# xiezhy6/PASTA-GAN-plusplus

Hardware: AMD Instinct MI355X
Metric: 512-res try-on images/sec (SynthesisNetwork fwd) (higher is better)
Workload: dtype f32

## Files before the change

### include/pasta_gan_ops.h

```cpp
#ifndef PASTA_GAN_OPS_H
#define PASTA_GAN_OPS_H

#include <stdint.h>

#ifdef __cplusplus
extern "C" {
#endif

#define PG_ABI_VERSION 19

enum pg_dtype { PG_F32 = 0, PG_F16 = 1, PG_BF16 = 2, PG_F64 = 3 };

enum pg_error {
    PG_OK = 0,
    PG_ERR_INVALID_ARG = -1,
    PG_ERR_UNSUPPORTED = -2,
    PG_ERR_TOO_LARGE = -3
};

enum pg_act {
    PG_ACT_LINEAR = 1, PG_ACT_RELU = 2, PG_ACT_LRELU = 3, PG_ACT_TANH = 4, PG_ACT_SIGMOID = 5,
    PG_ACT_ELU = 6, PG_ACT_SELU = 7, PG_ACT_SOFTPLUS = 8, PG_ACT_SWISH = 9
};

int pg_bias_act(const void* x, const void* b, const void* xref, const void* yref, const void* dy, void* y,
                int dtype, int64_t sizeX, int sizeB, int64_t stepB,
                int grad, int act, float alpha, float gain, float clamp, void* stream);
int pg_bias_act_abi_version(void);

int64_t pg_bias_act_grad_bias_workspace(int dtype, int64_t sizeX, int sizeB, int64_t stepB);
int pg_bias_act_grad_bias(const void* dy, const void* yref, void* dx, void* db, void* workspace, int64_t workspace_bytes,
                          int dtype, int64_t sizeX, int sizeB, int64_t stepB,
                          int act, float alpha, float gain, float clamp, void* stream);

int pg_upfirdn2d(const void* x, const float* f, void* y, int dtype,
                 int N, int C, int inH, int inW, const int64_t xstride[4],
                 int fh, int fw, const int64_t fstride[2],
                 int outH, int outW, const int64_t ystride[4],
                 int upx, int upy, int downx, int downy, int padx0, int pady0,
                 int flip, float gain, void* stream);
int pg_upfirdn2d_with_odd_samples(const void* x, const float* f, void* y, float* y_odd, int dtype,
                                  int N, int C, int inH, int inW, const int64_t xstride[4],
// ... 78 lines not shown
int pg_modconv_prep(const float* w2, const float* styles, float* out, float* s_norm, void* s16, int half_dtype,
                    int N, int Cout, int Cin, int normalize, int demodulate, void* stream);

#define PG_MODCONV_PREP_MAX_JOBS 32
typedef struct {
    const float* w2[PG_MODCONV_PREP_MAX_JOBS];
    const float* styles[PG_MODCONV_PREP_MAX_JOBS];
    float*       out[PG_MODCONV_PREP_MAX_JOBS];
    float*       s_norm[PG_MODCONV_PREP_MAX_JOBS];
    void*        s16[PG_MODCONV_PREP_MAX_JOBS];
    int          cout[PG_MODCONV_PREP_MAX_JOBS];
    int          cin[PG_MODCONV_PREP_MAX_JOBS];
    int          flags[PG_MODCONV_PREP_MAX_JOBS];
    int          njobs;
    int          half_dtype;
} pg_modconv_prep_jobs;
int pg_modconv_prep_batched(const pg_modconv_prep_jobs* jobs, int N, void* stream);

int pg_conv2d_up2_forward(const float* x, const float* packed, float* y, int N, int Cin, int H, int W, int Cout,
                          const int64_t ystride[4], const float* in_scale, const float* out_scale, void* stream);
int pg_conv2d_up2_splitk_plan(int N, int Cin, int H, int W, int Cout);
int pg_conv2d_up2_forward_splitk(const float* x, const float* packed, float* y, int N, int Cin, int H, int W, int Cout,
                                 const int64_t ystride[4], const float* in_scale, const float* out_scale, float* workspace, int ksplit, void* stream);

int64_t pg_conv2d_up2x3_packed_size(int Cout, int Cin);
int pg_conv2d_up2x3_pack_weight(const float* packed, void* packed_x3, int Cout, int Cin, void* stream);
int pg_conv2d_up2x3_forward(const float* x, const float* packed, const void* packed_x3, float* y, int N, int Cin, int H, int W, int Cout,
                            const int64_t ystride[4], const float* in_scale, const float* out_scale, float* edge_column, void* stream);

int64_t pg_conv2d_stem7x3_packed_size(int Cout);
int pg_conv2d_stem7x3_pack_weight(const float* w, void* packed, int Cout, float scale, int flip_hw, void* stream);
int pg_conv2d_stem7x3_forward(const float* x, const void* packed, float* y, int N, int H, int W, int Cout, const int64_t ystride[4],
                              const pg_conv2d_fusion* fusion, void* stream);

int pg_conv1x1_small(const float* x, const float* w, const float* styles, const float* bias, const float* skip, float* y,
                     int N, int Cin, int64_t HW, int Cout, float scale, float clamp, void* stream);

int pg_conv1x1_fold_prep(const float* wm, const float* bm, const float* wh, const float* bh, const float* styles, float* w_out, float* b_out,
                         int N, int Cm, int C, int Cout, void* stream);
int pg_conv1x1_fold_heads(const float* x, const float* x2, const float* w, const float* bias, const float* skip, float* y_a, float* y_b,
                          int N, int C1, int C2, int64_t HW, int Cout, int c_a, int n_skip, float clamp, void* stream);

int pg_conv3x3_fold_head(const float* xa, const float* xb, const float* w, const float* bias, const float* skip, float* y,
                         int N, int C, int H, int W, int Cout, float clamp, void* stream);

int pg_conv3x3_cin1(const float* x, const float* w, float* y, int N, int H, int W, int Cout, float scale, int act, void* stream);

int pg_instance_norm_stats(const float* x, float* mean, float* rstd, int NC, int64_t HW, float eps, void* stream);
int pg_spade_norm(const float* x, const float* mean, const float* rstd, const float* gamma, const float* beta,
                  float* y, int NC, int64_t HW, void* stream);

#define PG_STATS16_MAX_CHUNKS 256
int pg_instance_norm_stats_cl16(const void* x, float* mean, float* rstd, float* workspace, int dtype, int N, int64_t HW, int C, float eps, void* stream);
int pg_spade_combine_cl16(const void* x, const float* mean, const float* rstd, const void* gamma_beta, void* y, int dtype, int N, int64_t HW, int C,
                          int act, float alpha, float gain, float clamp, void* stream);

int pg_spade_train_forward(const float* x, const float* mean, const float* rstd, const float* gamma, const float* beta, float* y,
                           int N, int C, int64_t HW, int64_t gamma_sample_stride, int64_t beta_sample_stride, void* stream);
int pg_spade_train_backward(const float* dy, const float* x, const float* mean, const float* rstd, const float* gamma, float* sums,
                            float* dx, float* dgamma, float* dbeta, int N, int C, int64_t HW,
                            int64_t gamma_sample_stride, int64_t dgamma_sample_stride, int64_t dbeta_sample_stride, void* stream);

int pg_spade_masked_sums(const float* feat, const float* mask, const float* denorm_mask, float* sums, float* counts,
                         int N, int C, int H, int W, void* stream);
int pg_spade_feat_assemble(const float* feat_upper, const float* feat_lower, const float* mask_upper, const float* mask_lower,
                           const float* denorm_mask_upper, const float* denorm_mask_lower,
// ... 251 lines not shown
```

### pasta-gan-plusplus_amd/torch_utils/custom_ops.py

```python

import concurrent.futures
import ctypes
import fcntl
import glob
import hashlib
import os
import re
import shutil
import subprocess
import sys

verbosity = 'brief'

CSRC_DIR = os.path.normpath(os.path.join(os.path.dirname(os.path.abspath(__file__)), '..', 'csrc'))
INCLUDE_DIR = os.path.normpath(os.path.join(CSRC_DIR, '..', '..', 'include'))
DEV_DIR = os.path.join(CSRC_DIR, 'dev')
OFFLOAD_ARCH = 'gfx950'
HIPCC_FLAGS = ['-O3', '-std=c++17', '-fPIC', '-fvisibility=hidden', f'--offload-arch={OFFLOAD_ARCH}']

PLUGIN_SOURCES = {
    'bias_act_plugin': ['bias_act.hip'],
    'upfirdn2d_plugin': ['upfirdn2d.hip'],
    'patch_routing_plugin': ['patch_routing.hip'],
    'augment_plugin': ['augment.hip'],
    'tryon_plugin': ['tryon.hip'],
    'tryon_front_plugin': ['tryon_front.hip'],
    'train_fetch_plugin': ['train_fetch.hip'],
    'snapshot_grid_plugin': ['snapshot_grid.hip'],
    'vgg_loss_plugin': ['vgg_loss.hip'],
    'image_metrics_plugin': ['image_metrics.hip'],
    'conv2d_plugin': ['conv2d.hip', 'conv2d_inst_k3s1.hip', 'conv2d_inst_k1s1.hip', 'conv2d_inst_k2x2.hip', 'conv2d_inst_k2x1.hip',
                      'conv2d_inst_k1x2.hip', 'conv2d_inst_k7s1.hip', 'conv2d_inst_k3s2.hip', 'conv2d_inst_k1s2.hip', 'conv2d_inst_wino.hip', 'conv2d_inst_wino4.hip', 'conv2d_inst_wino4s.hip', 'conv2d_inst_wino4t.hip', 'conv2d_inst_wino4x.hip', 'conv2d_inst_wino4xs.hip', 'conv2d_inst_wino4xt.hip', 'conv2d_inst_wino4b.hip', 'conv2d_inst_wino4bs.hip', 'conv2d_inst_up2.hip', 'conv2d_inst_stem7.hip', 'conv2d_inst_s1x1.hip',
                      'conv2d_wgrad.hip', 'conv2d16.hip', 'conv2d16_inst_k3s1.hip', 'conv2d16_inst_k3s1b.hip', 'conv2d16_inst_k1s1.hip', 'conv2d16_inst_k2x2.hip', 'conv2d16_inst_k2x1.hip',
                      'conv2d16_inst_k1x2.hip', 'conv2d16_inst_k3s2.hip', 'conv2d16_inst_up2f.hip', 'conv1x1_head16.hip', 'spade16.hip', 'conv1x1_fold.hip', 'conv3x3_fold.hip', 'optim.hip'],
}

ABI_VERSION = 19

_cached_plugins = dict()


class NativePlugin:

    def __init__(self, name, path, abi_name=None):
        self.name = name
        self.path = path
        self.lib = ctypes.CDLL(path)
        probe = getattr(self.lib, 'pg_' + (abi_name or name).replace('_plugin', '') + '_abi_version', None)
        if probe is None:
            raise RuntimeError(f'{path} does not export its ABI version; rebuild it from csrc/')
        probe.restype = ctypes.c_int
        if probe() != ABI_VERSION:
            raise RuntimeError(f'{path} implements ABI version {probe()}, the bindings expect {ABI_VERSION}; rebuild it from csrc/')

    def __repr__(self):
        return f'<NativePlugin {self.name} at {self.path}>'


def _find_hipcc():
    for cand in (os.environ.get('HIPCC'), shutil.which('hipcc'), '/opt/rocm/bin/hipcc'):
        if cand and os.path.isfile(cand):
            return cand
    return None


def _digest(sources, extra_flags):
    h = hashlib.md5()
    deps = sorted(set(list(sources) + glob.glob(os.path.join(CSRC_DIR, '*.h')) + glob.glob(os.path.join(INCLUDE_DIR, '*.h'))))
    for path in deps:
        h.update(os.path.basename(path).encode())
# ... 180 lines not shown
```

### pasta-gan-plusplus_amd/torch_utils/ops/conv2d_gradfix.py

```python

import contextlib
import os

import weakref

import torch

from . import _native as nat
from . import bias_act
from . import conv2d_mfma
from . import conv2d_mfma16

native_input_gradients = os.environ.get('PG_NATIVE_DGRAD', '1') == '1'
native_weight_gradients16 = os.environ.get('PG_NATIVE_WGRAD16', '1') == '1'
native_weight_gradients = os.environ.get('PG_NATIVE_WGRAD', '1') == '1'
enabled = True
weight_gradients_disabled = False


@contextlib.contextmanager
def no_weight_gradients():
    global weight_gradients_disabled
    old = weight_gradients_disabled
    weight_gradients_disabled = True
# ... 117 lines not shown
    if hit is None:
        w = weight.detach()
        if not w.is_contiguous():
            w = w.contiguous()
        hit = conv2d_mfma.pack_weight(w, flip=flip, transpose_oi=transpose_oi, winograd=winograd)
        if sum(e[1].numel() * e[1].element_size() for e in _pack_cache.values()) + hit.numel() * hit.element_size() > _PACK_CACHE_MAX_BYTES:
            _pack_cache.clear()

        def _evict(ref, key=key):
            e = _pack_cache.get(key)
            if e is not None and e[0] is ref:
                del _pack_cache[key]
        _pack_cache[key] = (weakref.ref(base, _evict), hit)
    return hit


def _epilogue_backward(ctx, dy, y, ep, want_b):
    act, alpha, gain, clamp = ep
    if want_b:
        return bias_act._BiasActGrad.apply(dy, None, None, y, 1, act, alpha, gain, clamp, True)
    return bias_act._BiasActGrad.apply(dy, None, None, y, 1, act, alpha, gain, clamp), None


class _Conv2dMfma(torch.autograd.Function):
    @staticmethod
    def forward(ctx, x, weight, bias, stride, padding, transposed, output_padding, ep=None):
        x = x.contiguous()
        n, cin, h, w = x.shape
        kh, kw = int(weight.shape[2]), int(weight.shape[3])
        if not transposed:
            cout = int(weight.shape[0])
            fz = dict(act=ep[0], alpha=ep[1], gain=ep[2], clamp=ep[3] if ep[3] >= 0 else None) if ep is not None else {}
            wg = conv2d_mfma.use_winograd(kh, kw, stride, cout, cin, pad=padding, hw=(h, w), ep=fz)
            y = conv2d_mfma.conv2d_forward(x, _packed(weight, wg), cout, kh, kw, stride=stride, pad=padding, bias=bias, winograd=wg, **fz)
        else:
            assert ep is None
            cout = int(weight.shape[1])
            out_hw = ((h - 1) * stride - 2 * padding[0] + kh + output_padding[0], (w - 1) * stride - 2 * padding[1] + kw + output_padding[1])
            if ((kh, kw, stride) == (3, 3, 2) and tuple(padding) == (0, 0) and tuple(output_padding) == (0, 0) and bias is None and UP2_TRANSPOSED
                    and (n * cout * out_hw[0] * ((out_hw[1] + 3) // 4 * 4)) * 4 < 2 ** 31):
                main = _packed(weight, 0, flip=False, transpose_oi=True)
                packs = dict(main=main)
                if UP2_TRANSPOSED_X3 and cin % 16 == 0 and cin >= 32:
                    hit = _x3_of_pack.get(id(main))
                    if hit is None or hit[0]() is not main:
                        x3 = conv2d_mfma.pack_s2x3_planes(main, cout, cin)
                        _x3_of_pack[id(main)] = hit = (weakref.ref(main, lambda r, k=id(main): _x3_of_pack.pop(k, None)), x3)
                    packs['x3'] = hit[1]
                y = conv2d_mfma.conv_up2_forward(x, packs, cout, x3=None if 'x3' in packs else False)
            else:
                phases = conv2d_mfma.pack_transposed(weight, stride, padding, (h, w), out_hw)
                y = conv2d_mfma.conv_transpose2d_forward(x, phases, cout, out_hw, stride=stride, bias=bias)
        ctx.save_for_backward(x, weight, y if ep is not None else None)
        ctx.cfg = (stride, padding, transposed, output_padding, bias is not None, ep)
        return y

    @staticmethod
    def backward(ctx, dy):
        x, weight, y = ctx.saved_tensors
        stride, padding, transposed, output_padding, has_bias, ep = ctx.cfg
        kh, kw = int(weight.shape[2]), int(weight.shape[3])
        dx = dw = db = None
        if ep is not None:
            dy, db = _epilogue_backward(ctx, dy, y, ep, has_bias and ctx.needs_input_grad[2])
        if ctx.needs_input_grad[0] and native_input_gradients:
            dx = _input_gradient(dy, x.shape, weight, stride, padding, transposed, output_padding)
        want_w = ctx.needs_input_grad[1] and not weight_gradients_disabled
# ... 138 lines not shown
```

### pasta-gan-plusplus_amd/torch_utils/ops/conv2d_mfma.py

```python

import contextlib
import ctypes
import os

import torch

from .. import custom_ops
from . import _native as nat

ACT_INDEX = {'linear': 1, 'relu': 2, 'lrelu': 3, 'tanh': 4, 'sigmoid': 5, 'elu': 6, 'selu': 7, 'softplus': 8, 'swish': 9}

FUSED_ACTS = ('linear', 'relu', 'lrelu')

SUPPORTED = {(3, 3, 1), (1, 1, 1), (2, 2, 1), (2, 1, 1), (1, 2, 1), (7, 7, 1), (3, 3, 2), (1, 1, 2)}


class Fusion(ctypes.Structure):
    _fields_ = [
        ('in_scale', ctypes.c_void_p), ('in_bias', ctypes.c_void_p), ('in_act', ctypes.c_int), ('in_alpha', ctypes.c_float),
        ('in_gain', ctypes.c_float), ('in_clamp', ctypes.c_float),
        ('out_scale', ctypes.c_void_p), ('noise', ctypes.c_void_p), ('noise_batch_stride', ctypes.c_int64), ('noise_gain', ctypes.c_float),
        ('bias', ctypes.c_void_p), ('act', ctypes.c_int), ('alpha', ctypes.c_float), ('gain', ctypes.c_float), ('clamp', ctypes.c_float),
        ('residual', ctypes.c_void_p),
        ('spade_x', ctypes.c_void_p), ('spade_mean', ctypes.c_void_p), ('spade_rstd', ctypes.c_void_p),
        ('x2', ctypes.c_void_p), ('cin_split', ctypes.c_int),
        ('stats_partial', ctypes.c_void_p),
    ]


_plugin = None

_timeline = None
_wgrad_timeline = None


def reserve_cus(n):
# ... 71 lines not shown
        lib.pg_spade_norm.argtypes = [vp, vp, vp, vp, vp, vp, i, i64, vp]
        lib.pg_spade_train_forward.restype = i
        lib.pg_spade_train_forward.argtypes = [vp] * 6 + [i, i, i64, i64, i64, vp]
        lib.pg_spade_train_backward.restype = i
        lib.pg_spade_train_backward.argtypes = [vp] * 9 + [i, i, i64, i64, i64, i64, vp]
        lib.pg_conv2d_wgrad_plan.restype = i
        lib.pg_conv2d_wgrad_plan.argtypes = [i] * 8
        lib.pg_conv2d_wgrad.restype = i
        lib.pg_conv2d_wgrad.argtypes = [vp, vp, vp, vp] + [i] * 13 + [vp]
        lib.pg_conv2d_up2_forward.restype = i
        lib.pg_conv2d_up2_forward.argtypes = [vp, vp, vp, i, i, i, i, i, ctypes.POINTER(ctypes.c_int64), vp, vp, vp]
        lib.pg_split3_bf16_cl.restype = i
        lib.pg_split3_bf16_cl.argtypes = [vp, vp, i, i, i64, vp]
        lib.pg_conv2d16_wgrad_x3.restype = i
        lib.pg_conv2d16_wgrad_x3.argtypes = [vp, vp, vp, vp] + [i] * 13 + [vp]
        lib.pg_conv2d16_wgrad_plan.restype = i
        lib.pg_conv2d16_wgrad_plan.argtypes = [i] * 8
        lib.pg_conv2d_up2_splitk_plan.restype = i
        lib.pg_conv2d_up2_splitk_plan.argtypes = [i, i, i, i, i]
        lib.pg_conv2d_up2x3_packed_size.restype = i64
        lib.pg_conv2d_up2x3_packed_size.argtypes = [i, i]
        lib.pg_conv2d_up2x3_pack_weight.restype = i
        lib.pg_conv2d_up2x3_pack_weight.argtypes = [vp, vp, i, i, vp]
        lib.pg_conv2d_up2x3_forward.restype = i
        lib.pg_conv2d_up2x3_forward.argtypes = [vp, vp, vp, vp, i, i, i, i, i, ctypes.POINTER(ctypes.c_int64), vp, vp, vp, vp]
        lib.pg_conv2d_up2_forward_splitk.restype = i
        lib.pg_conv2d_up2_forward_splitk.argtypes = [vp, vp, vp, i, i, i, i, i, ctypes.POINTER(ctypes.c_int64), vp, vp, vp, i, vp]
        lib.pg_conv2d_stem7x3_packed_size.restype = i64
        lib.pg_conv2d_stem7x3_packed_size.argtypes = [i]
        lib.pg_conv2d_stem7x3_pack_weight.restype = i
        lib.pg_conv2d_stem7x3_pack_weight.argtypes = [vp, vp, i, ctypes.c_float, i, vp]
        lib.pg_conv2d_stem7x3_forward.restype = i
        lib.pg_conv2d_stem7x3_forward.argtypes = [vp, vp, vp, i, i, i, i, ctypes.POINTER(ctypes.c_int64), ctypes.POINTER(Fusion), vp]
        lib.pg_conv3x3_cin1.restype = i
        lib.pg_conv3x3_cin1.argtypes = [vp, vp, vp, i, i, i, i, f, i, vp]
        lib.pg_conv1x1_small.restype = i
        lib.pg_conv1x1_small.argtypes = [vp] * 6 + [i, i, i64, i, f, f, vp]
        lib.pg_conv1x1_fold_prep.restype = i
        lib.pg_conv1x1_fold_prep.argtypes = [vp] * 7 + [i, i, i, i, vp]
        lib.pg_conv1x1_fold_heads.restype = i
        lib.pg_conv1x1_fold_heads.argtypes = [vp] * 7 + [i, i, i, i64, i, i, i, f, vp]
        lib.pg_conv3x3_fold_head.restype = i
        lib.pg_conv3x3_fold_head.argtypes = [vp] * 6 + [i, i, i, i, i, f, vp]
        _plugin = plugin
    return _plugin


WINO_F2, WINO_F4, WINO_F4B, WINO_F4X3 = 1, 2, 3, 4
WINO_FORMS = {0: ('direct', False, False), WINO_F2: ('winograd', False, False), WINO_F4: ('winograd4', True, False),
              WINO_F4B: ('winograd4', False, True), WINO_F4X3: ('winograd4x3', True, False)}


def _wino_form(winograd):
    if int(winograd) not in WINO_FORMS:
        raise nat.NativeOpError(f'conv2d_mfma: winograd={winograd!r} is not one of the forms {sorted(WINO_FORMS)}')
    return (int(winograd), *WINO_FORMS[int(winograd)])


_WINO4B = os.environ.get('PG_WINO4B', '1')
F4_FORM = WINO_F4 if _WINO4B == '0' else WINO_F4B
F4_WIDE = WINO_F4 if os.environ.get('PG_WINO4_X3', '1') == '0' else WINO_F4X3


def f4_form(hw):
    if _WINO4B == '2':
        return WINO_F4B
# ... 46 lines not shown


def _f32c(t, name):
    if t is None:
        return None
    if t.dtype != torch.float32 or not t.is_cuda:
        raise nat.NativeOpError(f'conv2d_mfma: {name} must be a float32 GPU tensor')
    return t.contiguous()


def pack_weight(w, scale=1.0, flip=False, transpose_oi=False, winograd=False):
    lib = _init().lib
    w = _f32c(w.detach(), 'weight')
    if transpose_oi:
        cin, cout, kh, kw = w.shape
    else:
        cout, cin, kh, kw = w.shape
    form = _wino_form(winograd)[0]
    if form:
        if (kh, kw) != (3, 3):
            raise nat.NativeOpError('conv2d_mfma: the Winograd layout is for 3x3 weights')
        packed = torch.empty([lib.pg_conv2d_winograd_packed_size(form, cout, cin)], dtype=torch.float32, device=w.device)
        with torch.cuda.device(w.device):
            st = lib.pg_conv2d_winograd_pack_weight(form, nat.ptr(w), nat.ptr(packed), cout, cin, float(scale), int(bool(flip)), int(bool(transpose_oi)), nat.stream_of(w))
        nat.check(st, 'pg_conv2d_winograd_pack_weight')
        return packed
    packed = torch.empty([lib.pg_conv2d_packed_size(cout, cin, kh, kw)], dtype=torch.float32, device=w.device)
    with torch.cuda.device(w.device):
        st = lib.pg_conv2d_pack_weight(nat.ptr(w), nat.ptr(packed), cout, cin, kh, kw, float(scale), int(bool(flip)), int(bool(transpose_oi)), nat.stream_of(w))
    nat.check(st, 'pg_conv2d_pack_weight')
    return packed


def conv2d_forward(x, packed, cout, kh, kw, stride=1, pad=(0, 0), out_hw=None, y=None, out_step=(1, 1), out_off=(0, 0),
                   in_scale=None, in_bias=None, in_act='linear', in_alpha=0.0, in_gain=1.0, in_clamp=None,
                   out_scale=None, noise=None, noise_gain=1.0, bias=None, act='linear', alpha=0.0, gain=1.0, clamp=None,
                   residual=None, spade=None, x2=None, winograd=False, stats_eps=None):
    lib = _init().lib
    form, label, has_stats_tail, _ = _wino_form(winograd)
    x = _f32c(x, 'x')
    n, cin, h, w = x.shape
    cin_split = 0
    if x2 is not None:
        x2 = _f32c(x2, 'x2')
        if x2.shape[0] != n or x2.shape[2:] != x.shape[2:] or cin % 16 != 0:
            raise nat.NativeOpError('conv2d_mfma: x2 must match x in N, H, W and x must have a multiple of 16 channels')
        cin_split, cin = cin, cin + x2.shape[1]
    pad_y, pad_x = pad
    if out_hw is None:
        out_hw = ((h + 2 * pad_y - kh) // stride + 1, (w + 2 * pad_x - kw) // stride + 1)
    oh, ow = out_hw
    ychan = cout // 2 if spade is not None else cout
    if y is None:
        assert tuple(out_step) == (1, 1) and tuple(out_off) == (0, 0)
        y = torch.empty([n, ychan, oh, ow], dtype=torch.float32, device=x.device)
    else:
        assert y.dtype == torch.float32 and y.device == x.device and y.shape[0] == n and y.shape[1] == ychan
    fz = Fusion()
    keep = []

    def dev(t, name, numel=None):
        t = _f32c(t, name)
        if t is None:
            return None
        if numel is not None and t.numel() != numel:
            raise nat.NativeOpError(f'conv2d_mfma: {name} has {t.numel()} elements, expected {numel}')
        keep.append(t)
        return t.data_ptr()

    fz.in_scale = dev(in_scale, 'in_scale', n * cin)
# ... 10 lines not shown
        else:
            raise nat.NativeOpError('conv2d_mfma: noise must have OH*OW or N*OH*OW elements')
        keep.append(noise)
        fz.noise = noise.data_ptr()
    fz.noise_gain = float(noise_gain)
    fz.bias = dev(bias, 'bias', cout)
    fz.act, fz.alpha, fz.gain = ACT_INDEX[act], float(alpha), float(gain)
    fz.clamp = -1.0 if clamp is None else float(clamp)
    if residual is not None:
        if residual.dtype != torch.float32 or residual.shape != y.shape or residual.stride() != y.stride():
            raise nat.NativeOpError('conv2d_mfma: residual must match y in dtype, shape and strides')
        keep.append(residual)
        fz.residual = residual.data_ptr()
    if spade is not None:
        sx, smean, srstd = spade
        if sx.dtype != torch.float32 or sx.shape != y.shape or sx.stride() != y.stride() or smean.numel() != n * ychan or srstd.numel() != n * ychan:
            raise nat.NativeOpError('conv2d_mfma: spade tensors must match the [N, C, OH, OW] output')
        keep += [sx, smean, srstd]
        fz.spade_x, fz.spade_mean, fz.spade_rstd = sx.data_ptr(), smean.data_ptr(), srstd.data_ptr()
    if x2 is not None:
        keep.append(x2)
        fz.x2, fz.cin_split = x2.data_ptr(), cin_split
    stats_part = None
    if stats_eps is not None:
        if not has_stats_tail or spade is not None or in_scale is not None or noise is not None or residual is not None or x2 is not None or in_act != 'linear':
            raise nat.NativeNotCovered('conv2d_mfma: output statistics are gathered by the F(4x4) kernel\'s plain tail only')
        stats_T = lib.pg_conv2d_winograd4_stats_tiles(int(oh), int(ow))
        stats_part = torch.empty([n * cout * stats_T * 2], dtype=torch.float32, device=x.device)
        fz.stats_partial = stats_part.data_ptr()
    with torch.cuda.device(x.device):
        if _timeline is not None:
            ev0, ev1 = torch.cuda.Event(enable_timing=True), torch.cuda.Event(enable_timing=True)
            ev0.record()
        if form:
            if (kh, kw, int(stride)) != (3, 3, 1) or tuple(out_step) != (1, 1) or tuple(out_off) != (0, 0):
                raise nat.NativeOpError('conv2d_mfma: winograd=True needs a 3x3 stride-1 dense-output launch')
            st = lib.pg_conv2d_winograd_forward(form, nat.ptr(x), nat.ptr(packed), nat.ptr(y), n, cin, h, w, cout, int(pad_y), int(pad_x),
                                                int(oh), int(ow), nat.i64arr(y.stride()), ctypes.byref(fz), nat.stream_of(x))
        else:
            ksplit = 1
            if spade is None and x2 is None and os.environ.get('PG_CONV_SPLITK', '1') != '0':
                ksplit = lib.pg_conv2d_splitk_plan(n, cin, int(oh), int(ow), cout, kh, kw, int(stride))
            if ksplit > 1:
                ws = torch.empty([ksplit * n * cout * int(oh) * int(ow)], dtype=torch.float32, device=x.device)
                st = lib.pg_conv2d_forward_splitk(nat.ptr(x), nat.ptr(packed), nat.ptr(y), n, cin, h, w, cout, kh, kw, int(stride), int(pad_y), int(pad_x),
                                                  int(oh), int(ow), nat.i64arr(y.stride()), int(out_step[0]), int(out_step[1]), int(out_off[0]), int(out_off[1]),
                                                  ctypes.byref(fz), nat.ptr(ws), ksplit, nat.stream_of(x))
            else:
                st = lib.pg_conv2d_forward(nat.ptr(x), nat.ptr(packed), nat.ptr(y), n, cin, h, w, cout, kh, kw, int(stride), int(pad_y), int(pad_x),
                                           int(oh), int(ow), nat.i64arr(y.stride()), int(out_step[0]), int(out_step[1]), int(out_off[0]), int(out_off[1]),
                                           ctypes.byref(fz), nat.stream_of(x))
        if _timeline is not None:
            ev1.record()
            _timeline.append(((kh, kw, int(stride), label, f'N{n} {cin}->{cout} {h}x{w}' + (' spade' if spade is not None else '') + (' xf' if in_act != 'linear' else '') + (' mod' if in_scale is not None else '') + (' res' if residual is not None else '')), 2.0 * n * cout * oh * ow * cin * kh * kw, ev0, ev1,
                              4 * (x.numel() + (x2.numel() if x2 is not None else 0) + n * ychan * oh * ow)))
    nat.check(st, 'pg_conv2d_forward')
    if stats_part is not None:
        mean = torch.empty([n * cout], dtype=torch.float32, device=x.device)
        rstd = torch.empty_like(mean)
        with torch.cuda.device(x.device):
            st = lib.pg_instance_norm_finish(nat.ptr(stats_part), nat.ptr(mean), nat.ptr(rstd), n * cout, stats_T, int(oh), int(ow), float(stats_eps), nat.stream_of(x))
        nat.check(st, 'pg_instance_norm_finish')
        return y, (mean, rstd)
    return y


def pack_spade_gamma_beta(w_gamma, w_beta, scale_gamma=1.0, scale_beta=1.0, winograd=False):
    c = int(w_gamma.shape[0])
    grp = 32
    assert w_gamma.shape == w_beta.shape and c % 32 == 0
    if _wino_form(winograd)[3]:
        gw, bw = w_gamma.detach() * scale_gamma, w_beta.detach() * scale_beta
        return pack_weight(torch.stack([gw, bw], dim=1).reshape(2 * c, *w_gamma.shape[1:]).contiguous(), winograd=winograd)
    g = (w_gamma.detach() * scale_gamma).reshape(c // grp, grp, *w_gamma.shape[1:])
    b = (w_beta.detach() * scale_beta).reshape(c // grp, grp, *w_beta.shape[1:])
    return pack_weight(torch.cat([g, b], dim=1).reshape(2 * c, *w_gamma.shape[1:]).contiguous(), winograd=winograd)


def transposed_phases(kh, kw, stride, pad_y, pad_x, in_hw, out_hw):
    s = stride

    def axis(k, pad, n_out):
        res = []
        for a in range(s):
            j = -(-(k - a) // s)
            if j <= 0:
                return None
# ... 521 lines not shown
```

Baseline: 285.0.

## Add warp-specialized bf16x3 MFMA kernel for 3x3 stride-2 unpadded convolutions

Adds a dedicated persistent kernel for 3x3 stride-2 pad-0 convolutions. Producer waves DMA input rows into LDS and split each fp32 value into three bf16 planes, while consumer waves run bf16 32x32x16 MFMAs over six plane products to emulate fp32 precision, with double-buffered planes and prefetched weight slabs. The goal is to move these convs from the generic fp32 path onto the matrix cores. It is used by default only in inference with no grad and simple epilogues, and falls back when unsupported. The bf16x3 split gives slightly different rounding than true fp32.

```diff
diff --git a/include/pasta_gan_ops.h b/include/pasta_gan_ops.h
--- a/include/pasta_gan_ops.h
+++ b/include/pasta_gan_ops.h
@@ -7,7 +7,7 @@
 extern "C" {
 #endif
 
-#define PG_ABI_VERSION 19
+#define PG_ABI_VERSION 20
 
 enum pg_dtype { PG_F32 = 0, PG_F16 = 1, PG_BF16 = 2, PG_F64 = 3 };
 
@@ -152,6 +152,11 @@
 int pg_conv2d_stem7x3_pack_weight(const float* w, void* packed, int Cout, float scale, int flip_hw, void* stream);
 int pg_conv2d_stem7x3_forward(const float* x, const void* packed, float* y, int N, int H, int W, int Cout, const int64_t ystride[4],
                               const pg_conv2d_fusion* fusion, void* stream);
+
+int64_t pg_conv2d_s2x3_packed_size(int Cout, int Cin);
+int pg_conv2d_s2x3_pack_weight(const float* packed, void* packed_x3, int Cout, int Cin, void* stream);
+int pg_conv2d_s2x3_forward(const float* x, const void* packed_x3, float* y, int N, int Cin, int H, int W, int Cout, const int64_t ystride[4],
+                           const pg_conv2d_fusion* fusion, void* stream);
 
 int pg_conv1x1_small(const float* x, const float* w, const float* styles, const float* bias, const float* skip, float* y,
                      int N, int Cin, int64_t HW, int Cout, float scale, float clamp, void* stream);
diff --git a/pasta-gan-plusplus_amd/csrc/conv2d_inst_s2x3.hip b/pasta-gan-plusplus_amd/csrc/conv2d_inst_s2x3.hip
--- /dev/null
+++ b/pasta-gan-plusplus_amd/csrc/conv2d_inst_s2x3.hip
@@ -0,0 +1,38 @@
+#include "conv2d_s2x3.h"
+
+PG_EXPORT int64_t pg_conv2d_s2x3_packed_size(int Cout, int Cin) {
+    if (Cout <= 0 || Cin <= 0 || Cin % 16 != 0) return 0;
+    return pgconv::s2x3_packed_bytes(Cout, Cin);
+}
+
+PG_EXPORT int pg_conv2d_s2x3_pack_weight(const float* packed, void* packed_x3, int Cout, int Cin, void* stream) {
+    if (!packed || !packed_x3 || Cout <= 0 || Cin <= 0 || (((uintptr_t)packed_x3) & 15) != 0) return PG_ERR_INVALID_ARG;
+    if (Cin % 16 != 0) return PG_ERR_UNSUPPORTED;
+    const int CoutP32 = (Cout + 31) / 32 * 32, CoutP128 = (Cout + 127) / 128 * 128;
+    const int64_t total = (int64_t)Cin * 9 * CoutP128;
+    int64_t blocks = (total + 255) / 256;
+    if (blocks > (int64_t)pg::max_stream_blocks()) blocks = pg::max_stream_blocks();
+    hipLaunchKernelGGL(pgconv::s2x3_pack_kernel, dim3((unsigned)blocks), dim3(256), 0, (hipStream_t)stream, packed, (unsigned short*)packed_x3, Cin, CoutP128, CoutP32);
+    return pg::launch_status();
+}
+
+PG_EXPORT int pg_conv2d_s2x3_forward(const float* x, const void* packed_x3, float* y, int N, int Cin, int H, int W, int Cout, const int64_t ystride[4],
+                                     const pg_conv2d_fusion* fusion, void* stream) {
+    if (!x || !packed_x3 || !y || !ystride || N <= 0 || Cin <= 0 || H <= 0 || W <= 0 || Cout <= 0) return PG_ERR_INVALID_ARG;
+    if ((((uintptr_t)x) & 3) != 0 || (((uintptr_t)packed_x3) & 15) != 0) return PG_ERR_INVALID_ARG;
+    pgconv::S2x3Params p;
+    p.x = x; p.y = y; p.wx3 = (const unsigned char*)packed_x3; p.bias = nullptr;
+    p.N = N; p.Cin = Cin; p.H = H; p.W = W; p.Cout = Cout;
+    for (int i = 0; i < 4; i++) p.ys[i] = ystride[i];
+    p.act = PG_ACT_LINEAR; p.alpha = 0.f; p.gain = 1.f; p.clamp = -1.f;
+    if (fusion) {
+        const pg_conv2d_fusion& f = *fusion;
+        if (f.in_scale || f.in_bias || (f.in_act != 0 && f.in_act != PG_ACT_LINEAR) || f.in_clamp >= 0.f || (f.in_gain != 0.f && f.in_gain != 1.f) || f.out_scale || f.noise || f.residual ||
+            f.spade_x || f.spade_mean || f.spade_rstd || f.x2 || f.stats_partial)
+            return PG_ERR_UNSUPPORTED;
+        const int act = f.act == 0 ? PG_ACT_LINEAR : f.act;
+        if (act != PG_ACT_LINEAR && act != PG_ACT_RELU && act != PG_ACT_LRELU) return PG_ERR_UNSUPPORTED;
+        p.bias = f.bias; p.act = act; p.alpha = f.alpha; p.gain = f.gain == 0.f ? 1.f : f.gain; p.clamp = f.clamp;
+    }
+    return pgconv::launch_s2x3(p, (hipStream_t)stream);
+}
diff --git a/pasta-gan-plusplus_amd/csrc/conv2d_s2x3.h b/pasta-gan-plusplus_amd/csrc/conv2d_s2x3.h
--- /dev/null
+++ b/pasta-gan-plusplus_amd/csrc/conv2d_s2x3.h
@@ -0,0 +1,353 @@
+#pragma once
+#include "conv2d_kernel.h"
+
+#ifndef SX_EXP
+#define SX_EXP 0
+#endif
+
+namespace pgconv {
+
+constexpr int SX_KC = 16;
+constexpr int SX_TH = 4, SX_TW = 16;
+constexpr int SX_IH = 9, SX_IW = 33;
+constexpr int SX_RW = 10;
+constexpr int SX_RAW = (512 + 3 * 320) * 4;
+constexpr int SX_PR = 34;
+constexpr int SX_NPIX = SX_IH * SX_PR;
+constexpr int SX_PLB = SX_NPIX * 32;
+constexpr int SX_GROUP = 128;
+constexpr int SX_FRAG = 64 * 16;
+constexpr int SX_WSLAB = 27 * SX_FRAG;
+constexpr size_t SX_LDS = (size_t)SX_RAW * 4 + 2 * 3 * (size_t)SX_PLB + 2 * SX_GROUP * 4;
+
+struct S2x3Params {
+    const float* x; float* y; const unsigned char* wx3; const float* bias;
+    int N, Cin, H, W, Cout, OH, OW;
+    int tilesX, tilesY, groups, total_tiles;
+    int64_t ys[4];
+    int act; float alpha, gain, clamp;
+};
+
+typedef __bf16 sx_bf16x8 __attribute__((ext_vector_type(8)));
+typedef unsigned sx_u32x4 __attribute__((ext_vector_type(4)));
+
+__device__ __forceinline__ void sx_split_pair(float va, float vb, unsigned& p0, unsigned& p1, unsigned& p2) {
+    const unsigned ua = __float_as_uint(va), ub = __float_as_uint(vb);
+    const float ra = va - __uint_as_float(ua & 0xffff0000u), rb = vb - __uint_as_float(ub & 0xffff0000u);
+    const unsigned ura = __float_as_uint(ra), urb = __float_as_uint(rb);
+    const float la = ra - __uint_as_float(ura & 0xffff0000u), lb = rb - __uint_as_float(urb & 0xffff0000u);
+    p0 = __builtin_amdgcn_perm(ub, ua, 0x07060302u);
+    p1 = __builtin_amdgcn_perm(urb, ura, 0x07060302u);
+    p2 = __builtin_amdgcn_perm(__float_as_uint(lb), __float_as_uint(la), 0x07060302u);
+}
+
+__global__ __launch_bounds__(512, 1) void conv2d_s2x3(S2x3Params p) {
+    extern __shared__ __attribute__((aligned(16))) unsigned char sx_smem[];
+    float* raw = (float*)sx_smem;
+    unsigned char* planes = sx_smem + SX_RAW * 4;
+    float* bias_s = (float*)(planes + 2 * 3 * SX_PLB);
+
+    const int wave = __builtin_amdgcn_readfirstlane((int)threadIdx.x >> 6);
+    const int lane = (int)threadIdx.x & 63;
+    const unsigned smem_b = __builtin_amdgcn_readfirstlane(lds_offset((const float*)sx_smem));
+    const int HW = p.H * p.W;
+    const int nchunks = p.Cin / SX_KC;
+    const int total = p.total_tiles;
+    const int q8 = total >> 3, r8 = total & 7;
+    const int my_tiles = (total - (int)blockIdx.x + (int)gridDim.x - 1) / (int)gridDim.x;
+    const int my_chunks = my_tiles * nchunks;
+
+    auto decode = [&](int tile, int& n, int& oy0, int& ox0, int& grp) __attribute__((always_inline)) {
+        const int xcd = tile & 7;
+        int L = (xcd < r8 ? xcd * (q8 + 1) : r8 * (q8 + 1) + (xcd - r8) * q8) + (tile >> 3);
+        grp = L % p.groups; L /= p.groups;
+        const int tx = L % p.tilesX; L /= p.tilesX;
+        const int ty = L % p.tilesY;
+        n = L / p.tilesY;
+        oy0 = ty * SX_TH; ox0 = tx * SX_TW;
+    };
+    auto image_base = [&](int n, int& delta) __attribute__((always_inline)) {
+        const uint64_t b = (uint64_t)(uintptr_t)(p.x + (int64_t)n * p.Cin * HW);
+        delta = (int)((b & 15u) >> 2);
+        return b & ~(uint64_t)15;
+    };
+
+    if (wave >= 4) {
+        const int pw = wave - 4;
+        const int nrows = pw == 0 ? 3 : 2;
+        const int nreq = pw == 0 ? 8 : 5;
+        const int reg_w = pw == 0 ? 0 : 512 + (pw - 1) * 320;
+        unsigned xoff[8];
+        i32x4 xrsrc;
+        int c_tile = blockIdx.x, c_chunk = 0;
+        int s_tile = blockIdx.x, s_chunk = 0, s_sb = 0, s_grp = 0, s_par = 0;
+        const int w3 = p.W & 3, hw3 = HW & 3;
+        auto request_rows = [&]() __attribute__((always_inline)) {
+            if (c_chunk == 0) {
+                int n, oy0, ox0, grp, delta;
+                decode(c_tile, n, oy0, ox0, grp);
+                const uint64_t base = image_base(n, delta);
+                const int gx0 = 2 * ox0;
+                const int ncols = p.W - gx0 < SX_IW ? p.W - gx0 : SX_IW;
+                int ll = lane;
+                asm volatile("" : "+v"(ll));
+#pragma unroll
+                for (int i = 0; i < 8; i++) {
+                    const int f = i * 64 + ll;
+                    const int ri = f / 160, rem = f % 160;
+                    const int c = rem / SX_RW, wd = rem % SX_RW;
+                    const int row = ri == 0 ? pw : (ri == 1 ? pw + 4 : 8);
+                    const int gy = 2 * oy0 + row;
+                    const int e0 = delta + c * HW + gy * p.W + gx0;
+                    const bool ok = ri < nrows && gy < p.H && 4 * wd < (e0 & 3) + ncols;
+                    xoff[i] = ok ? (unsigned)((e0 & ~3) + 4 * wd) * 4u : 0x80000000u;
+                }
+                xrsrc[0] = (int)(unsigned)base;
+                xrsrc[1] = (int)(unsigned)(base >> 32) & 0xffff;
+                xrsrc[2] = (p.Cin * HW + 4) * 4;
+                xrsrc[3] = 0x00020000;
+            }
+            i32x4 rs;
+#pragma unroll
+            for (int i = 0; i < 4; i++) rs[i] = __builtin_amdgcn_readfirstlane(xrsrc[i]);
+            const unsigned xs_b = smem_b + (unsigned)reg_w * 16u;
+            const int soff = c_chunk * SX_KC * HW * 4;
+#pragma unroll
+            for (int i = 0; i < 8; i++)
+                if (i < nreq && !(SX_EXP & 4)) dma_dwordx4_buf(rs, xs_b + 1024u * i, xoff[i], soff);
+            if (++c_chunk == nchunks) { c_chunk = 0; c_tile += gridDim.x; }
+        };
+        auto split_rows = [&](int g) __attribute__((always_inline)) {
+            if (s_chunk == 0) {
+                int n, oy0, ox0, delta;
+                decode(s_tile, n, oy0, ox0, s_grp);
+                image_base(n, delta);
+                s_sb = (delta + ((2 * oy0) & 3) * w3) & 3;
+            }
+            if (pw == 0 && s_chunk + 1 == nchunks) {
+#pragma unroll
+                for (int h = 0; h < 2; h++) {
+                    const int co = s_grp * SX_GROUP + 64 * h + lane;
+                    bias_s[s_par * SX_GROUP + 64 * h + lane] = (p.bias && co < p.Cout) ? ld_opaque(p.bias + co) : 0.f;
+                }
+            }
+            unsigned char* pl_b = planes + (size_t)(g & 1) * 3 * SX_PLB;
+#pragma unroll
+            for (int i = 0; i < 4; i++) {
+                const int task = lane + 64 * i;
+                if (task < nrows * 66) {
+                    const int ri = task / 66, rem = task - ri * 66;
+                    const int kh = rem >= SX_IW ? 1 : 0, col = rem - SX_IW * kh;
+                    const int row = ri == 0 ? pw : (ri == 1 ? pw + 4 : 8);
+                    const int sh_row = s_sb + (row & 3) * w3;
+                    const float* rp = raw + (reg_w + ri * 160 + (8 * kh) * SX_RW) * 4 + col;
+                    sx_u32x4 pl[3];
+#pragma unroll
+                    for (int j = 0; j < 4; j++) {
+                        const int ca = 8 * kh + 2 * j, cb = ca + 1;
+                        const float va = rp[ca % 8 * 40 + ((sh_row + ca * hw3) & 3)], vb = rp[cb % 8 * 40 + ((sh_row + cb * hw3) & 3)];
+                        unsigned p0, p1, p2;
+                        if (SX_EXP & 2) { p0 = __float_as_uint(va); p1 = __float_as_uint(vb); p2 = p0; }
+                        else sx_split_pair(va, vb, p0, p1, p2);
+                        pl[0][j] = p0; pl[1][j] = p1; pl[2][j] = p2;
+                    }
+                    unsigned char* dst = pl_b + (size_t)(kh * SX_NPIX + row * SX_PR + (col & 1) * 17 + (col >> 1)) * 16;
+                    *(sx_u32x4*)(dst) = pl[0];
+                    *(sx_u32x4*)(dst + SX_PLB) = pl[1];
+                    *(sx_u32x4*)(dst + 2 * SX_PLB) = pl[2];
+                }
+            }
+            if (++s_chunk == nchunks) { s_chunk = 0; s_tile += gridDim.x; s_par ^= 1; }
+        };
+        request_rows();
+        for (int g = 0; g < my_chunks; g++) {
+            asm volatile("s_waitcnt vmcnt(0)" ::: "memory");
+            split_rows(g);
+            asm volatile("s_waitcnt lgkmcnt(0)" ::: "memory");
+            if (g + 1 < my_chunks) request_rows();
+            asm volatile("s_barrier" ::: "memory");
+        }
+        asm volatile("s_barrier" ::: "memory");
+        return;
+    }
+
+    const int half = lane >> 5, l31 = lane & 31;
+    const int orow = l31 >> 4, ocol = l31 & 15;
+    f32x16 acc[2], accs[2];
+    sx_u32x4 A[9][3];
+    auto wslab = [&](int grp, int chunk) __attribute__((always_inline)) {
+        return p.wx3 + (((int64_t)grp * nchunks + chunk) * 4 + wave) * (int64_t)SX_WSLAB + lane * 16;
+    };
+    int tile = blockIdx.x, par = 0;
+    int e_n, e_oy0, e_ox0, e_grp;
+    decode(tile, e_n, e_oy0, e_ox0, e_grp);
+    {
+        const unsigned char* w0 = wslab(e_grp, 0);
+#pragma unroll
+        for (int t = 0; t < 9; t++)
+#pragma unroll
+            for (int pl = 0; pl < 3; pl++) A[t][pl] = (SX_EXP & 8) ? (sx_u32x4){0u, 0u, 0u, 0u} : *(const sx_u32x4*)(w0 + (t * 3 + pl) * SX_FRAG);
+        __builtin_amdgcn_s_waitcnt(0x0f70);
+#pragma unroll
+        for (int t = 0; t < 9; t++)
+#pragma unroll
+            for (int pl = 0; pl < 3; pl++) asm volatile("" : "+v"(A[t][pl]));
+    }
+    unsigned long long st_mm = 0, st_bar = 0, st_ep = 0, st_t0 = 0, st_rounds = 0;
+    const float gain = p.gain;
+    const float cl = p.clamp >= 0.f ? p.clamp : __builtin_inff();
+    const float slope = act_slope(p.act, p.alpha);
+    const int cs_ = (int)p.ys[1], rs_ = (int)p.ys[2], xs_ = (int)p.ys[3];
+    asm volatile("s_barrier" ::: "memory");
+    for (int ti = 0, g = 0; ti < my_tiles; ti++, par ^= 1) {
+#pragma unroll
+        for (int a = 0; a < 2; a++)
+#pragma unroll
+            for (int k = 0; k < 16; k++) acc[a][k] = accs[a][k] = 0.f;
+        int nx_n = e_n, nx_oy0 = e_oy0, nx_ox0 = e_ox0, nx_grp = e_grp;
+        if (ti + 1 < my_tiles) decode(tile + (int)gridDim.x, nx_n, nx_oy0, nx_ox0, nx_grp);
+        for (int k = 0; k < nchunks; k++, g++) {
+            const int wb = g & 1;
+            if (SX_EXP & 32) st_t0 = __builtin_amdgcn_s_memtime();
+            const unsigned char* wn = k + 1 < nchunks ? wslab(e_grp, k + 1) : wslab(nx_grp, 0);
+            {
+                const unsigned char* bb = planes + (size_t)wb * 3 * SX_PLB + (size_t)(half * SX_NPIX + 2 * orow * SX_PR + ocol) * 16;
+                auto b_frag = [&](int t, int a, int pl) __attribute__((always_inline)) {
+                    const int ky = t / 3, kx = t % 3;
+                    return *(const sx_u32x4*)(bb + (size_t)pl * SX_PLB + (size_t)((4 * a + ky) * SX_PR + (kx & 1) * 17 + (kx >> 1)) * 16);
+                };
+                constexpr int PA[6] = {2, 1, 1, 0, 0, 0}, PB[6] = {0, 1, 0, 2, 1, 0};
+                sx_u32x4 B[2][3];
+                f32x16 accp[2];
+#pragma unroll
+                for (int a = 0; a < 2; a++)
+#pragma unroll
+                    for (int k = 0; k < 16; k++) accp[a][k] = 0.f;
+#pragma unroll
+                for (int pl = 0; pl < 3; pl++) B[0][pl] = b_frag(0, 0, pl);
+#pragma unroll
+                for (int t = 0; t < 9; t++) {
+#pragma unroll
+                    for (int a = 0; a < 2; a++) {
+                        if (a == 0 || t + 1 < 9) {
+#pragma unroll
+                            for (int pl = 0; pl < 3; pl++) B[a ^ 1][pl] = a == 0 ? b_frag(t, 1, pl) : b_frag(t + 1, 0, pl);
+                        }
+                        __builtin_amdgcn_sched_barrier(0);
+#pragma unroll
+                        for (int pr = 0; pr < 6; pr++) {
+                            f32x16& dacc = pr == 5 ? accp[a] : accs[a];
+                            if (!(SX_EXP & 1) || A[t][PA[pr]][0] == 0x12345678u)
+                                dacc = __builtin_amdgcn_mfma_f32_32x32x16_bf16(__builtin_bit_cast(sx_bf16x8, A[t][PA[pr]]), __builtin_bit_cast(sx_bf16x8, B[a][PB[pr]]), dacc, 0, 0, 0);
+                        }
+                        __builtin_amdgcn_sched_barrier(0);
+                    }
+                    if (!(SX_EXP & 8)) {
+#pragma unroll
+                        for (int pl = 0; pl < 3; pl++) A[t][pl] = *(const sx_u32x4*)(wn + (t * 3 + pl) * SX_FRAG);
+                    }
+                    __builtin_amdgcn_sched_barrier(0);
+                }
+#pragma unroll
+                for (int a = 0; a < 2; a++)
+#pragma unroll
+                    for (int k = 0; k < 16; k++) acc[a][k] += accp[a][k];
+            }
+            if (SX_EXP & 32) { const unsigned long long t1 = __builtin_amdgcn_s_memtime(); st_mm += t1 - st_t0; st_t0 = t1; }
+            asm volatile("s_waitcnt lgkmcnt(0)\n\ts_barrier" ::: "memory");
+            if (SX_EXP & 32) { st_bar += __builtin_amdgcn_s_memtime() - st_t0; st_rounds++; }
+        }
+
+        if (SX_EXP & 32) st_t0 = __builtin_amdgcn_s_memtime();
+        {
+            int ll;
+            asm volatile("v_mbcnt_lo_u32_b32 %0, -1, 0\n\tv_mbcnt_hi_u32_b32 %0, -1, %0" : "=v"(ll));
+            const int half = ll >> 5, orow = (ll >> 4) & 1, ocol = ll & 15;
+            const int ox = e_ox0 + ocol;
+            const int co0 = e_grp * SX_GROUP + 32 * wave + 4 * half;
+            i32x4 yrsrc;
+            {
+                const uint64_t base = (uint64_t)(uintptr_t)(p.y + (int64_t)e_n * p.ys[0]);
+                yrsrc[0] = __builtin_amdgcn_readfirstlane((int)(unsigned)base);
+                yrsrc[1] = __builtin_amdgcn_readfirstlane((int)(unsigned)(base >> 32) & 0xffff);
+                yrsrc[2] = 0x7ffffffc;
+                yrsrc[3] = 0x00020000;
+            }
+            const float* bs = bias_s + par * SX_GROUP + 32 * wave + 4 * half;
+#pragma unroll
+            for (int kq = 0; kq < 4; kq++) {
+                const f32x4 b4 = *(const f32x4*)(bs + 8 * kq);
+#pragma unroll
+                for (int a = 0; a < 2; a++) {
+                    const int oy = e_oy0 + 2 * a + orow;
+                    const bool ok = oy < p.OH && ox < p.OW;
+                    const unsigned o0 = (unsigned)((co0 + 8 * kq) * cs_ + oy * rs_ + ox * xs_) * 4u;
+#pragma unroll
+                    for (int j = 0; j < 4; j++) {
+                        float v = (acc[a][4 * kq + j] + accs[a][4 * kq + j]) + b4[j];
+                        v = v > 0.f ? v : v * slope;
+                        v = fminf(fmaxf(v * gain, -cl), cl);
+                        const unsigned off = (ok && co0 + 8 * kq + j < p.Cout && (!(SX_EXP & 16) || v == 12345.678f)) ? o0 + (unsigned)(j * cs_) * 4u : 0x80000000u;
+                        asm volatile("buffer_store_dword %0, %1, %2, 0 offen" :: "v"(v), "v"(off), "s"(yrsrc) : "memory");
+                    }
+                }
+            }
+        }
+        if (SX_EXP & 32) st_ep += __builtin_amdgcn_s_memtime() - st_t0;
+        tile += gridDim.x;
+        e_n = nx_n; e_oy0 = nx_oy0; e_ox0 = nx_ox0; e_grp = nx_grp;
+    }
+    if (SX_EXP & 32) {
+        asm volatile("s_waitcnt vmcnt(0)" ::: "memory");
+        if (blockIdx.x == 0 && lane == 0) {
+            unsigned long long* o = (unsigned long long*)p.y + wave * 4;
+            o[0] = st_mm; o[1] = st_bar; o[2] = st_ep; o[3] = st_rounds;
+        }
+    }
+}
+
+__global__ __launch_bounds__(256) void s2x3_pack_kernel(const float* __restrict__ wp32, unsigned short* __restrict__ out, int Cin, int CoutP128, int CoutP32) {
+    const int nchunks = Cin / SX_KC;
+    const int64_t total = (int64_t)Cin * 9 * CoutP128;
+    for (int64_t i = (int64_t)blockIdx.x * 256 + threadIdx.x; i < total; i += (int64_t)gridDim.x * 256) {
+        const int co = (int)(i % CoutP128), tap = (int)((i / CoutP128) % 9), ci = (int)(i / ((int64_t)CoutP128 * 9));
+        const float v = co < CoutP32 ? wp32[((int64_t)ci * 9 + tap) * CoutP32 + co] : 0.f;
+        const unsigned u0 = __float_as_uint(v) & 0xffff0000u;
+        const float r = v - __uint_as_float(u0);
+        const unsigned u1 = __float_as_uint(r) & 0xffff0000u;
+        const unsigned u2 = __float_as_uint(r - __uint_as_float(u1)) & 0xffff0000u;
+        const int grp = co >> 7, mb = (co >> 5) & 3, m = co & 31, chunk = ci >> 4, kh = (ci >> 3) & 1, j = ci & 7;
+        const int64_t dst = ((((((int64_t)grp * nchunks + chunk) * 4 + mb) * 9 + tap) * 3) * 2 + kh) * 256 + m * 8 + j;
+        out[dst] = (unsigned short)(u0 >> 16);
+        out[dst + 512] = (unsigned short)(u1 >> 16);
+        out[dst + 1024] = (unsigned short)(u2 >> 16);
+    }
+}
+
+inline int64_t s2x3_packed_bytes(int Cout, int Cin) { return (int64_t)((Cout + SX_GROUP - 1) / SX_GROUP) * (Cin / SX_KC) * 4 * SX_WSLAB; }
+
+inline bool s2x3_serves(const S2x3Params& p) {
+    return p.H >= 3 && p.W >= 3 && p.Cin % SX_KC == 0 && p.Cin >= 2 * SX_KC && (((uintptr_t)p.x) & 3) == 0 &&
+           ((int64_t)p.Cin * p.H * p.W + 4) * 4 < 0x7fffffffLL;
+}
+
+inline int launch_s2x3(S2x3Params p, hipStream_t s) {
+    if (!s2x3_serves(p) || !p.wx3) return PG_ERR_UNSUPPORTED;
+    p.OH = (p.H - 3) / 2 + 1; p.OW = (p.W - 3) / 2 + 1;
+    p.tilesX = (p.OW + SX_TW - 1) / SX_TW;
+    p.tilesY = (p.OH + SX_TH - 1) / SX_TH;
+    p.groups = (p.Cout + SX_GROUP - 1) / SX_GROUP;
+    const int64_t tiles = (int64_t)p.N * p.tilesX * p.tilesY * p.groups;
+    if (tiles > 0x7fffffffLL) return PG_ERR_TOO_LARGE;
+    if (((int64_t)(p.groups * SX_GROUP) * p.ys[1] + (int64_t)p.OH * p.ys[2] + (int64_t)p.OW * p.ys[3]) * 4 >= 0x7fffffffLL) return PG_ERR_UNSUPPORTED;
+    if (p.ys[1] < 0 || p.ys[2] < 0 || p.ys[3] < 0) return PG_ERR_UNSUPPORTED;
+    p.total_tiles = (int)tiles;
+    const int64_t blocks = tiles < (int64_t)num_cu() ? tiles : (int64_t)num_cu();
+    static PerDeviceOnce once;
+    const hipError_t e = once.run([] { return hipFuncSetAttribute((const void*)conv2d_s2x3, hipFuncAttributeMaxDynamicSharedMemorySize, 160 * 1024); });
+    if (e != hipSuccess) return (int)e;
+    hipLaunchKernelGGL(conv2d_s2x3, dim3((unsigned)blocks), dim3(512), SX_LDS, s, p);
+    return launch_status();
+}
+
+}
diff --git a/pasta-gan-plusplus_amd/torch_utils/custom_ops.py b/pasta-gan-plusplus_amd/torch_utils/custom_ops.py
--- a/pasta-gan-plusplus_amd/torch_utils/custom_ops.py
+++ b/pasta-gan-plusplus_amd/torch_utils/custom_ops.py
@@ -30,12 +30,12 @@
     'vgg_loss_plugin': ['vgg_loss.hip'],
     'image_metrics_plugin': ['image_metrics.hip'],
     'conv2d_plugin': ['conv2d.hip', 'conv2d_inst_k3s1.hip', 'conv2d_inst_k1s1.hip', 'conv2d_inst_k2x2.hip', 'conv2d_inst_k2x1.hip',
-                      'conv2d_inst_k1x2.hip', 'conv2d_inst_k7s1.hip', 'conv2d_inst_k3s2.hip', 'conv2d_inst_k1s2.hip', 'conv2d_inst_wino.hip', 'conv2d_inst_wino4.hip', 'conv2d_inst_wino4s.hip', 'conv2d_inst_wino4t.hip', 'conv2d_inst_wino4x.hip', 'conv2d_inst_wino4xs.hip', 'conv2d_inst_wino4xt.hip', 'conv2d_inst_wino4b.hip', 'conv2d_inst_wino4bs.hip', 'conv2d_inst_up2.hip', 'conv2d_inst_stem7.hip', 'conv2d_inst_s1x1.hip',
+                      'conv2d_inst_k1x2.hip', 'conv2d_inst_k7s1.hip', 'conv2d_inst_k3s2.hip', 'conv2d_inst_k1s2.hip', 'conv2d_inst_wino.hip', 'conv2d_inst_wino4.hip', 'conv2d_inst_wino4s.hip', 'conv2d_inst_wino4t.hip', 'conv2d_inst_wino4x.hip', 'conv2d_inst_wino4xs.hip', 'conv2d_inst_wino4xt.hip', 'conv2d_inst_wino4b.hip', 'conv2d_inst_wino4bs.hip', 'conv2d_inst_up2.hip', 'conv2d_inst_stem7.hip', 'conv2d_inst_s2x3.hip', 'conv2d_inst_s1x1.hip',
                       'conv2d_wgrad.hip', 'conv2d16.hip', 'conv2d16_inst_k3s1.hip', 'conv2d16_inst_k3s1b.hip', 'conv2d16_inst_k1s1.hip', 'conv2d16_inst_k2x2.hip', 'conv2d16_inst_k2x1.hip',
                       'conv2d16_inst_k1x2.hip', 'conv2d16_inst_k3s2.hip', 'conv2d16_inst_up2f.hip', 'conv1x1_head16.hip', 'spade16.hip', 'conv1x1_fold.hip', 'conv3x3_fold.hip', 'optim.hip'],
 }
 
-ABI_VERSION = 19
+ABI_VERSION = 20
 
 _cached_plugins = dict()
 
diff --git a/pasta-gan-plusplus_amd/torch_utils/ops/conv2d_gradfix.py b/pasta-gan-plusplus_amd/torch_utils/ops/conv2d_gradfix.py
--- a/pasta-gan-plusplus_amd/torch_utils/ops/conv2d_gradfix.py
+++ b/pasta-gan-plusplus_amd/torch_utils/ops/conv2d_gradfix.py
@@ -173,7 +173,7 @@
             cout = int(weight.shape[0])
             fz = dict(act=ep[0], alpha=ep[1], gain=ep[2], clamp=ep[3] if ep[3] >= 0 else None) if ep is not None else {}
             wg = conv2d_mfma.use_winograd(kh, kw, stride, cout, cin, pad=padding, hw=(h, w), ep=fz)
-            y = conv2d_mfma.conv2d_forward(x, _packed(weight, wg), cout, kh, kw, stride=stride, pad=padding, bias=bias, winograd=wg, **fz)
+            y = conv2d_mfma.conv2d_forward(x, _packed(weight, wg), cout, kh, kw, stride=stride, pad=padding, bias=bias, winograd=wg, s2x3=False, **fz)
         else:
             assert ep is None
             cout = int(weight.shape[1])
diff --git a/pasta-gan-plusplus_amd/torch_utils/ops/conv2d_mfma.py b/pasta-gan-plusplus_amd/torch_utils/ops/conv2d_mfma.py
--- a/pasta-gan-plusplus_amd/torch_utils/ops/conv2d_mfma.py
+++ b/pasta-gan-plusplus_amd/torch_utils/ops/conv2d_mfma.py
@@ -2,6 +2,7 @@
 import contextlib
 import ctypes
 import os
+import weakref
 
 import torch
 
@@ -139,6 +140,12 @@
         lib.pg_conv2d_stem7x3_pack_weight.argtypes = [vp, vp, i, ctypes.c_float, i, vp]
         lib.pg_conv2d_stem7x3_forward.restype = i
         lib.pg_conv2d_stem7x3_forward.argtypes = [vp, vp, vp, i, i, i, i, ctypes.POINTER(ctypes.c_int64), ctypes.POINTER(Fusion), vp]
+        lib.pg_conv2d_s2x3_packed_size.restype = i64
+        lib.pg_conv2d_s2x3_packed_size.argtypes = [i, i]
+        lib.pg_conv2d_s2x3_pack_weight.restype = i
+        lib.pg_conv2d_s2x3_pack_weight.argtypes = [vp, vp, i, i, vp]
+        lib.pg_conv2d_s2x3_forward.restype = i
+        lib.pg_conv2d_s2x3_forward.argtypes = [vp, vp, vp, i, i, i, i, i, ctypes.POINTER(i64), ctypes.POINTER(Fusion), vp]
         lib.pg_conv3x3_cin1.restype = i
         lib.pg_conv3x3_cin1.argtypes = [vp, vp, vp, i, i, i, i, f, i, vp]
         lib.pg_conv1x1_small.restype = i
@@ -251,10 +258,32 @@
     return packed
 
 
+S2_X3 = os.environ.get('PG_S2_X3', '1') != '0'
+_s2x3_of_pack = {}
+
+
+def s2x3_wanted(n, cin, cout, h, w):
+    if not S2_X3 or os.environ.get('PG_S2_X3', '1') == '0' or cin % 16 != 0 or cin < 32 or h < 3 or w < 3:
+        return False
+    return True
+
+
+def pack_s2x3(packed32, cout, cin):
+    hit = _s2x3_of_pack.get(id(packed32))
+    if hit is not None and hit[0]() is packed32:
+        return hit[1]
+    lib = _init().lib
+    x3 = torch.empty([lib.pg_conv2d_s2x3_packed_size(cout, cin)], dtype=torch.uint8, device=packed32.device)
+    with torch.cuda.device(packed32.device):
+        nat.check(lib.pg_conv2d_s2x3_pack_weight(nat.ptr(packed32), nat.ptr(x3), cout, cin, nat.stream_of(packed32)), 'pg_conv2d_s2x3_pack_weight')
+    _s2x3_of_pack[id(packed32)] = (weakref.ref(packed32, lambda r, k=id(packed32): _s2x3_of_pack.pop(k, None)), x3)
+    return x3
+
+
 def conv2d_forward(x, packed, cout, kh, kw, stride=1, pad=(0, 0), out_hw=None, y=None, out_step=(1, 1), out_off=(0, 0),
                    in_scale=None, in_bias=None, in_act='linear', in_alpha=0.0, in_gain=1.0, in_clamp=None,
                    out_scale=None, noise=None, noise_gain=1.0, bias=None, act='linear', alpha=0.0, gain=1.0, clamp=None,
-                   residual=None, spade=None, x2=None, winograd=False, stats_eps=None):
+                   residual=None, spade=None, x2=None, winograd=False, stats_eps=None, s2x3=None):
     lib = _init().lib
     form, label, has_stats_tail, _ = _wino_form(winograd)
     x = _f32c(x, 'x')
@@ -331,7 +360,17 @@
         if _timeline is not None:
             ev0, ev1 = torch.cuda.Event(enable_timing=True), torch.cuda.Event(enable_timing=True)
             ev0.record()
-        if form:
+        s2x3 = (s2x3 is not False and not form and (kh, kw, int(stride)) == (3, 3, 2) and (int(pad_y), int(pad_x)) == (0, 0) and tuple(out_step) == (1, 1) and tuple(out_off) == (0, 0)
+                and (int(oh), int(ow)) == ((h - 3) // 2 + 1, (w - 3) // 2 + 1) and not torch.is_grad_enabled() and residual is None and spade is None and x2 is None
+                and in_scale is None and in_bias is None and out_scale is None and noise is None and in_act == 'linear' and float(in_gain) == 1.0 and in_clamp is None
+                and act in FUSED_ACTS and s2x3_wanted(n, cin, cout, h, w))
+        st = -2
+        if s2x3:
+            st = lib.pg_conv2d_s2x3_forward(nat.ptr(x), nat.ptr(pack_s2x3(packed, cout, cin)), nat.ptr(y), n, cin, h, w, cout, nat.i64arr(y.stride()), ctypes.byref(fz), nat.stream_of(x))
+            s2x3 = st != -2
+        if s2x3:
+            pass
+        elif form:
             if (kh, kw, int(stride)) != (3, 3, 1) or tuple(out_step) != (1, 1) or tuple(out_off) != (0, 0):
                 raise nat.NativeOpError('conv2d_mfma: winograd=True needs a 3x3 stride-1 dense-output launch')
             st = lib.pg_conv2d_winograd_forward(form, nat.ptr(x), nat.ptr(packed), nat.ptr(y), n, cin, h, w, cout, int(pad_y), int(pad_x),
@@ -351,7 +390,7 @@
                                            ctypes.byref(fz), nat.stream_of(x))
         if _timeline is not None:
             ev1.record()
-            _timeline.append(((kh, kw, int(stride), label, f'N{n} {cin}->{cout} {h}x{w}' + (' spade' if spade is not None else '') + (' xf' if in_act != 'linear' else '') + (' mod' if in_scale is not None else '') + (' res' if residual is not None else '')), 2.0 * n * cout * oh * ow * cin * kh * kw, ev0, ev1,
+            _timeline.append(((kh, kw, int(stride), label, f'N{n} {cin}->{cout} {h}x{w}' + (' spade' if spade is not None else '') + (' xf' if in_act != 'linear' else '') + (' mod' if in_scale is not None else '') + (' res' if residual is not None else '') + (' s2x3' if s2x3 else '')), 2.0 * n * cout * oh * ow * cin * kh * kw, ev0, ev1,
                               4 * (x.numel() + (x2.numel() if x2 is not None else 0) + n * ychan * oh * ow)))
     nat.check(st, 'pg_conv2d_forward')
     if stats_part is not None:
```

Result: faster. 288.1, median of 6 (+1.1%).
